# libnxz/power-gzip

Hardware: AMD Instinct MI355X
Metric: GiB/s uncompressed in (deflate), real-data corpus in 64 KiB blocks, exact dynamic-Huffman table per block (higher is better)
Workload: dtype u8

## Files before the change

### power-gzip_amd/csrc/nxz_batch.cpp

```cpp
#include "nxz_ctx.h"
#include "nxz_inflate_part.h"

static size_t compress_chunk(size_t n)
{
	static const size_t v = [] { const char *e = getenv("NXZ_COMPRESS_CHUNK"); size_t x = e ? (size_t)strtoull(e, nullptr, 0) : 0; return x >= 256 ? x : (size_t)0; }();
	if (v) return v;
	size_t c = 8192;
	while (c < 65536 && n >= 8 * c) c *= 2;
	return c;
}

static constexpr unsigned JOB_COUNTERS = 256;
#define NXZ_LANES_MIN 49152
static_assert(NXZ_INFLATE_PART_CHUNK_STREAMS < NXZ_LANES_MIN, "a chunk of nxz_batch_inflate_streams_part must stay below the batches that are sampled or go a stream per lane");
#define NXZ_LANES_TABLES_MIN 163840
#define NXZ_WINDOW_LDS_MAX 1024
#define NXZ_DICT_WG_MIN_DEFAULT 4096

extern "C" int nxz_dict_create(nxz_ctx_t *c, const uint8_t *bytes, size_t len, nxz_dict_t **out)
{
	if (!c || !out || (len && !bytes)) return -EINVAL;
	if (forked_child()) return -ENODEV;
	(void)hipSetDevice(c->device);
	nxz_dict *d = new (std::nothrow) nxz_dict;
	if (!d) return -ENOMEM;
	d->device = c->device; d->len = len;
	d->id = nxz_dict_adler32(bytes, len);
	d->win = nxz_dict_inflate_window(len); d->W = nxz_dict_deflate_window(len);
	std::vector<uint8_t> img(NXZ_DICT_WINDOW, 0);
	if (d->win) memcpy(img.data() + NXZ_DICT_WINDOW - d->win, bytes + nxz_dict_inflate_start(len), d->win);
	if (hipMalloc((void **)&d->d_win, NXZ_DICT_WINDOW) != hipSuccess) { (void)hipGetLastError(); delete d; return -ENOMEM; }
	hipError_t e = hipMemcpy(d->d_win, img.data(), NXZ_DICT_WINDOW, hipMemcpyHostToDevice);
	if (e != hipSuccess) { set_err("dictionary copy", e); (void)hipFree(d->d_win); delete d; return -EIO; }
	*out = d;
	return 0;
}
extern "C" void nxz_dict_destroy(nxz_ctx_t *c, nxz_dict_t *d)
{
	if (!d) return;
	if (!forked_child()) { (void)hipSetDevice(d->device); (void)hipFree(d->d_win); }
	delete d;
}
extern "C" uint32_t nxz_dict_id(const nxz_dict_t *d) { return d ? d->id : 1; }

static int batch_compress(nxz_ctx_t *c, int fc, const nxz_batch_job_t *jobs, size_t n,
			  const nxz_batch_dht_t *dht, size_t ntables, nxz_batch_result_t *results,
			  uint32_t *counts, void *stream, const nxz_dict *dict, const uint8_t *win = nullptr, size_t nwin = 0);
extern "C" int nxz_batch_compress(nxz_ctx_t *c, int fc, const nxz_batch_job_t *jobs, size_t n,
				  const nxz_batch_dht_t *dht, size_t ntables, nxz_batch_result_t *results,
				  uint32_t *counts, void *stream)
{
	return batch_compress(c, fc, jobs, n, dht, ntables, results, counts, stream, nullptr);
}
extern "C" int nxz_batch_compress_dict(nxz_ctx_t *c, int fc, const nxz_dict_t *dict, const nxz_batch_job_t *jobs, size_t n,
				       const nxz_batch_dht_t *dht, size_t ntables, nxz_batch_result_t *results,
				       uint32_t *counts, void *stream)
{
	if (!c || !dict || dict->device != c->device || n >= (1u << 31) || (n && (!jobs || !results))) return -EINVAL;
	return batch_compress(c, fc, jobs, n, dht, ntables, results, counts, stream, dict);
}
int batch_compress_windowed(nxz_ctx_t *c, int fc, const uint8_t *win, size_t nwin, const nxz_batch_job_t *jobs, size_t n,
			    nxz_batch_result_t *results, void *stream)
{
	if (!win || nwin > n) return -EINVAL;
	return batch_compress(c, fc, jobs, n, nullptr, 0, results, nullptr, stream, nullptr, win, nwin);
}
static int batch_compress(nxz_ctx_t *c, int fc, const nxz_batch_job_t *ujobs, size_t n,
			  const nxz_batch_dht_t *dht, size_t ntables, nxz_batch_result_t *results,
			  uint32_t *counts, void *stream, const nxz_dict *dict, const uint8_t *win, size_t nwin)
{
	const nxz_batch_job_t *jobs = ujobs;
	if (!c || !nxz_fc_is_compress((uint32_t)fc) || (fc & 1) || (fc & ~0x2e)) return -EINVAL;
	if (forked_child()) return -ENODEV;
	const bool gen = nxz_fc_is_dhtgen((uint32_t)fc);
	const bool isdht = nxz_fc_is_dht((uint32_t)fc), count = nxz_fc_has_count((uint32_t)fc);
	if (gen && !isdht) return -EINVAL;
	if (count && !counts) return -EINVAL;
	if (isdht && !gen && (!dht || !ntables)) return -EINVAL;
	if (n == 0) return 0;
	hipStream_t s = (hipStream_t)stream;
	(void)hipSetDevice(c->device);
	nxz_dht_prepared_t *prepared = nullptr;
	const char *fge = getenv("NXZ_FUSED_GEN");
	const bool fused_gen_on = fge && atoi(fge) != 0;
	const bool fused_gen = gen && fused_gen_on;
	const bool fused = (!isdht && !count) || fused_gen;
	size_t want = compress_chunk(n);
	size_t nchunks = fused ? 1 : (n + want - 1) / want;
	size_t chunk = (n + nchunks - 1) / nchunks;
	nxz_ctx::Scratch sc;
	const auto use = lease_scratch(c, s);
	const int sized = with_scratch(c, s, [&](nxz_ctx::Scratch &r) -> int {
		if (!fused && r.chunk_limit && want > r.chunk_limit) {
			want = r.chunk_limit; nchunks = (n + want - 1) / want; chunk = (n + nchunks - 1) / nchunks;
		}
		if (!fused && r.chunk_cap < chunk) {
			if (r.d_tokens) { (void)hipStreamSynchronize(s); r.release_chunk(); }
			const size_t per_job = (size_t)NXZ_TOK_STRIDE + sizeof(nxz_dht_prepared_t) + 316 * sizeof(uint32_t);
			size_t free_b = 0, total_b = 0;
			if (hipMemGetInfo(&free_b, &total_b) == hipSuccess && want > 8192 && chunk * per_job > free_b / 4) {
				while (want > 8192 && want * per_job > free_b / 4) want /= 2;
				nchunks = (n + want - 1) / want; chunk = (n + nchunks - 1) / nchunks;
				r.chunk_limit = want;
			}
			while (!r.alloc_chunk(chunk)) {
				if (want <= 1024) return -ENOMEM;
				want = want > 8192 ? 8192 : want / 2;
				nchunks = (n + want - 1) / want; chunk = (n + nchunks - 1) / nchunks;
				r.chunk_limit = want;
			}
		}
		if (!r.d_cand2) HIPCHK(hipMalloc((void **)&r.d_cand2, nxz_lz77_cand2_bytes()), return -ENOMEM);
		if (fused_gen && !r.d_fuse) HIPCHK(hipMalloc((void **)&r.d_fuse, nxz_lz77_gen_scratch_bytes()), return -ENOMEM);
		if (isdht && !gen && r.buf[BUF_PREPARED].grow(s, ntables * sizeof(nxz_dht_prepared_t)) == DevBuf::FAILED) return -ENOMEM;
		if (!c->d_job_counters && hipMalloc((void **)&c->d_job_counters, JOB_COUNTERS * sizeof(uint32_t)) != hipSuccess) c->d_job_counters = nullptr;
		if (dict && r.buf[BUF_DICT_JOBS].grow(s, n * sizeof(nxz_batch_job_t)) == DevBuf::FAILED) return -ENOMEM;
		sc = r;
		return 0;
	});
	if (sized) return sized;
	if (dict) {
		nxz_batch_job_t *djobs = sc.buf[BUF_DICT_JOBS].as<nxz_batch_job_t>();
		if (int rc = launched("dictionary jobs launch", nxz_launch_dict_jobs(ujobs, n, dict->W, djobs, s))) return rc;
		jobs = djobs;
	}
	if (isdht && !gen) {
		prepared = sc.buf[BUF_PREPARED].as<nxz_dht_prepared_t>();
		if (int rc = launched("dht prepare launch", nxz_launch_dht_prepare(dht, ntables, prepared, s))) return rc;
	}
	if (dict) { win = dict->deflate_window(); nwin = n; }
	for (size_t off = 0; off < n; off += chunk) {
		const size_t m = n - off < chunk ? n - off : chunk;
		const size_t mw = off < nwin ? std::min(m, nwin - off) : 0;
		auto draw = [&]() {
			std::lock_guard<std::mutex> g(c->mtx);
			return c->d_job_counters ? c->d_job_counters + (c->next_counter++ % JOB_COUNTERS) : nullptr;
		};
		uint32_t *cnt = count ? counts + off * 316 : gen ? sc.d_counts : nullptr;
		auto stamp = [&]() {
			if (!c->timing) return;
			hipEvent_t e;
			if (hipEventCreate(&e) != hipSuccess) return;
			(void)hipEventRecord(e, s);
			std::lock_guard<std::mutex> g(c->mtx);
			c->tev.push_back(e);
		};
		stamp();
		const int mode = fused_gen ? NXZ_LZ77_FUSED_GEN : fused ? NXZ_LZ77_FUSED_FHT : cnt != nullptr;
		uint8_t *const lz_scratch = fused_gen ? sc.d_fuse : sc.d_tokens;
		uint32_t *const lz_counts = fused_gen && !count ? nullptr : cnt;
		int rc = mw ? nxz_launch_lz77_dict(mode, jobs + off, mw, lz_scratch, sc.d_cand2, results + off, lz_counts, draw(), win, s) : 0;
		if (!rc && mw < m)
			rc = nxz_launch_lz77(mode, jobs + off + mw, m - mw, fused ? lz_scratch : lz_scratch + mw * (size_t)NXZ_TOK_STRIDE, sc.d_cand2,
					     results + off + mw, lz_counts ? lz_counts + mw * 316 : nullptr, draw(), s);
		if ((rc = launched("lz77 launch", rc)) != 0) return rc;
		stamp();
		if (fused) { stamp(); stamp(); continue; }
		if (gen) {
			if ((rc = launched("dhtgen launch", nxz_launch_dhtgen(cnt, m, sc.d_gen, nullptr, s))) != 0) return rc;
		}
		stamp();
		rc = launched("encode launch", nxz_launch_encode(isdht, gen, jobs + off, m, sc.d_tokens, gen ? sc.d_gen : prepared, results + off, s));
		if (rc) return rc;
		stamp();
	}
	return dict ? launched("dictionary finish launch", nxz_launch_dict_finish(ujobs, n, dict->W, results, s)) : 0;
}

size_t trim_compress_scratch()
{
	size_t freed = 0;
	std::lock_guard<std::mutex> g(g_mtx);
	for (nxz_ctx *c : g_ctx) {
		if (!c) continue;
		(void)hipSetDevice(c->device);
		std::vector<std::pair<hipStream_t, std::mutex *>> streams;
		{
			std::lock_guard<std::mutex> g2(c->mtx);
			for (auto &kv : c->scratch) streams.emplace_back(kv.first, &c->scratch_use[kv.first]);
		}
		for (auto &sm : streams) {
			if (!sm.second->try_lock()) continue;
			bool there;
			{
				std::lock_guard<std::mutex> g2(c->mtx);
				there = c->scratch.find(sm.first) != c->scratch.end();
			}
			if (there && hipStreamSynchronize(sm.first) != hipSuccess) { (void)hipGetLastError(); there = false; }
			if (there) {
				std::lock_guard<std::mutex> g2(c->mtx);
				auto it = c->scratch.find(sm.first);
				if (it != c->scratch.end()) {
					nxz_ctx::Scratch &r = it->second;
					if (r.d_tokens) freed += r.chunk_cap * ((size_t)NXZ_TOK_STRIDE + sizeof(nxz_dht_prepared_t) + 316 * sizeof(uint32_t));
					r.release_chunk();
					r.chunk_limit = 0;
				}
			}
			sm.second->unlock();
		}
	}
	return freed;
}

extern "C" void nxz_ctx_stage_timing(nxz_ctx_t *c, int on)
{
	if (!c) return;
	std::lock_guard<std::mutex> g(c->mtx);
	c->timing = on != 0;
}

extern "C" int nxz_ctx_stage_ms(nxz_ctx_t *c, double ms[3], unsigned *launches)
{
	if (!c || !ms) return -EINVAL;
	std::vector<hipEvent_t> ev;
	{
		std::lock_guard<std::mutex> g(c->mtx);
		ev.swap(c->tev);
	}
	ms[0] = ms[1] = ms[2] = 0;
	if (launches) *launches = (unsigned)(ev.size() / 4);
	for (size_t i = 0; i + 3 < ev.size(); i += 4) {
		(void)hipEventSynchronize(ev[i + 3]);
		for (int k = 0; k < 3; k++) {
			float f = 0;
			if (hipEventElapsedTime(&f, ev[i + k], ev[i + k + 1]) == hipSuccess) ms[k] += f;
		}
	}
	for (auto e : ev) (void)hipEventDestroy(e);
	return 0;
}

extern "C" int nxz_batch_dhtgen(nxz_ctx_t *c, const uint32_t *counts, size_t n, nxz_batch_dht_t *tables, void *stream)
{
	if (!c || !counts || !tables) return -EINVAL;
	if (forked_child()) return -ENODEV;
	(void)hipSetDevice(c->device);
	return launched("dhtgen launch", nxz_launch_dhtgen(counts, n, nullptr, tables, (hipStream_t)stream));
}

extern "C" int nxz_batch_decompress(nxz_ctx_t *c, const nxz_batch_job_t *jobs, size_t n,
// ... 238 lines not shown
```

### power-gzip_amd/csrc/nxz_device.h

```cpp
#ifndef NXZ_DEVICE_H
#define NXZ_DEVICE_H
#include <stdint.h>
#include <stddef.h>
#include "../../include/nxz_engine.h"

typedef struct nxz_dht_prepared {
	uint32_t dhtlen;
	uint32_t status;
	uint32_t dhtw[74];
	uint32_t ll[288];
	uint32_t d[32];
} nxz_dht_prepared_t;

#define NXZ_TOK_LITBITS    0u
#define NXZ_TOK_MATCHBITS  8192u
#define NXZ_TOK_RECORDS    16384u
#define NXZ_TOK_STRIDE     106496u
#define NXZ_TOK_MAXREC     ((NXZ_TOK_STRIDE - NXZ_TOK_RECORDS) / 4u)

#ifdef __HIPCC__
#include <hip/hip_runtime.h>
#define NXZ_GLOBAL_AS __attribute__((address_space(1)))
extern "C" {
#define NXZ_LZ77_MAX_GRID 512
#define NXZ_LZ77_FUSED_FHT 2
#define NXZ_LZ77_FUSED_GEN 3
size_t nxz_lz77_cand2_bytes(void);
size_t nxz_lz77_gen_scratch_bytes(void);
int nxz_launch_lz77(int count, const nxz_batch_job_t *jobs, size_t n, uint8_t *tokens, uint16_t *cand2, nxz_batch_result_t *results,
		    uint32_t *counts, uint32_t *job_counter, hipStream_t stream);
int nxz_launch_symcount(const nxz_batch_job_t *jobs, size_t n, const uint8_t *tokens, uint32_t *counts, hipStream_t stream);
int nxz_launch_encode(int dht, int table_per_job, const nxz_batch_job_t *jobs, size_t n, const uint8_t *tokens,
		      const nxz_dht_prepared_t *tables, nxz_batch_result_t *results, hipStream_t stream);
int nxz_launch_dhtgen(const uint32_t *counts, size_t n, nxz_dht_prepared_t *prepared,
		      nxz_batch_dht_t *tables, hipStream_t stream);
int nxz_launch_dht_prepare(const nxz_batch_dht_t *dht, size_t n, nxz_dht_prepared_t *out, hipStream_t stream);
int nxz_launch_wrap(const nxz_batch_job_t *jobs, size_t n, nxz_batch_result_t *results, hipStream_t stream);
int nxz_launch_wrap_sliced(const nxz_batch_job_t *jobs, size_t n, nxz_batch_result_t *results, hipStream_t stream);
int nxz_launch_inflate(const nxz_batch_job_t *jobs, size_t n, nxz_batch_result_t *results,
		       nxz_batch_dht_t *dht_io, int window_in_lds, const uint32_t *order, hipStream_t stream);
size_t nxz_order_workspace(size_t n);
const uint32_t *nxz_launch_order_by_length(const nxz_batch_job_t *jobs, size_t n, uint8_t *workspace, hipStream_t stream);
typedef struct nxz_sync_req {
	const uint8_t *src;
	uint32_t srclen;
	uint32_t header_bit;
	uint32_t guess_bit;
	uint32_t limit_bit;
} nxz_sync_req_t;
typedef struct nxz_sync_res { uint32_t bit; uint32_t lanes; } nxz_sync_res_t;
size_t nxz_built_tables_bytes(void);
#define NXZ_BLOCKFIND_MORE 3u
int nxz_launch_token_sync_more(const nxz_sync_req_t *breqs, uint32_t nb, nxz_batch_dht_t *tables, void *built, uint32_t first,
			       const nxz_sync_req_t *reqs, uint32_t n, nxz_sync_res_t *res, hipStream_t stream);
int nxz_launch_token_sync(const nxz_sync_req_t *breqs, uint32_t nb, nxz_batch_dht_t *tables, void *built,
			  const nxz_sync_req_t *reqs, uint32_t n, nxz_sync_res_t *res, hipStream_t stream);
typedef struct nxz_walk_req { const uint8_t *src; uint64_t src_len; uint64_t bit; uint32_t rem, bfinal; } nxz_walk_req_t;
typedef struct nxz_walk_res { uint64_t bit; uint32_t flags, reserved; } nxz_walk_res_t;
int nxz_launch_stored_walk(const nxz_walk_req_t *reqs, uint32_t n, nxz_walk_res_t *res, hipStream_t stream);
int nxz_launch_inflate_w16(const nxz_batch_job_t *jobs, size_t n, nxz_batch_result_t *results, nxz_batch_dht_t *dht_io, const void *built,
			   int few_and_even, hipStream_t stream);
int nxz_launch_sample_btype(const nxz_batch_job_t *jobs, size_t n, uint32_t *out, hipStream_t stream);
int nxz_launch_cksum(const nxz_batch_job_t *jobs, size_t n, nxz_batch_result_t *results, hipStream_t stream);
int nxz_launch_pack_stream(const nxz_batch_job_t *jobs, const nxz_batch_result_t *results, size_t n, uint32_t final_index,
			   uint64_t *offsets, uint8_t *packed, hipStream_t stream);
typedef struct nxz_pack_member { uint32_t b0, n, fin, off0; uint8_t *packed; } nxz_pack_member_t;
int nxz_launch_pack_member_streams(const nxz_batch_job_t *jobs, const nxz_batch_result_t *results, size_t nblocks, const nxz_pack_member_t *members,
				   size_t nmembers, const uint16_t *member_of, uint64_t *offsets, hipStream_t stream);
int nxz_launch_copy_items(const void *items, uint32_t n, hipStream_t stream);
int nxz_launch_copy16(const void *src, void *dst, size_t bytes, hipStream_t stream);
size_t nxz_inflate_lanes_workspace(size_t n);
unsigned nxz_inflate_cut_pieces(size_t n);
size_t nxz_inflate_cut_workspace(size_t n, unsigned pieces, size_t arena);
int nxz_launch_copy_out(const nxz_batch_job_t *jobs, const nxz_batch_result_t *results, uint8_t *const *targets, size_t n, hipStream_t stream);
int nxz_launch_inflate_cut(const nxz_batch_job_t *jobs, size_t n, nxz_batch_result_t *results, nxz_batch_dht_t *dht_io,
			   unsigned pieces, uint8_t *workspace, size_t arena, hipStream_t stream);
int nxz_launch_pack_members(const nxz_batch_job_t *jobs, const nxz_batch_result_t *results, size_t n,
			    uint64_t *offsets, uint8_t *packed, hipStream_t stream);
int nxz_launch_pack_zlib(const nxz_batch_job_t *jobs, const nxz_batch_result_t *results, size_t n, uint32_t flg,
			 uint64_t *offsets, uint8_t *packed, hipStream_t stream);
int nxz_launch_frame_header(int fmt, const nxz_batch_job_t *jobs, size_t n, nxz_batch_frame_t *frames, nxz_batch_job_t *derived, hipStream_t stream);
int nxz_launch_frame_trailer(const nxz_batch_job_t *jobs, size_t n, nxz_batch_result_t *results, nxz_batch_frame_t *frames, hipStream_t stream);
size_t nxz_bgzf_workspace(uint64_t len, uint64_t cap);
int nxz_launch_bgzf_discover(const uint8_t *packed, uint64_t len, uint8_t *dst, uint64_t *offsets, uint64_t max_members, uint8_t *ws,
			     uint64_t cap, nxz_batch_job_t **jobs, hipStream_t stream);
int nxz_launch_bgzf_coff(const uint8_t *packed, uint64_t len, uint8_t *ws, uint64_t cap, uint64_t max_members, uint64_t *coff, hipStream_t stream);
size_t nxz_bgzf_ranges_workspace(uint64_t n, uint64_t L);
int nxz_launch_bgzf_map(const uint8_t *packed, uint64_t packed_len, const uint64_t *coff, const uint64_t *uoff, uint64_t L, int kind,
			const nxz_bgzf_range_t *ranges, uint64_t n, uint64_t *offsets, uint32_t *status, uint8_t *ws, hipStream_t stream);
int nxz_launch_range_map_clear(uint8_t *ws, uint64_t n, uint64_t L, hipStream_t stream);
int nxz_launch_range_map_ranges(const uint64_t *uoff, uint64_t L, const nxz_bgzf_range_t *ranges, uint64_t n, uint64_t *offsets,
				uint32_t *status, uint8_t *ws, hipStream_t stream);
void nxz_range_map_lists(uint8_t *ws, uint64_t n, uint64_t L, const uint32_t **midx, const uint32_t **list);
int nxz_launch_bgzf_jobs(const uint8_t *packed, const uint64_t *coff, const uint64_t *uoff, uint64_t n, uint64_t L, uint8_t *ws,
			 uint64_t k0, uint64_t cnt, uint8_t *slots, uint64_t stride, nxz_batch_job_t *jobs, hipStream_t stream);
int nxz_launch_bgzf_gather(const uint64_t *uoff, uint64_t n, uint64_t L, uint64_t pieces, uint8_t *ws, const uint64_t *offsets,
			   const uint8_t *slots, uint64_t stride, uint64_t k0, uint64_t cnt, const nxz_batch_frame_t *frames,
			   const nxz_batch_result_t *results, uint8_t *dst, uint32_t *status, hipStream_t stream);
int nxz_launch_bgzf_zero(uint64_t n, const uint64_t *offsets, const uint32_t *status, uint8_t *dst, hipStream_t stream);
int nxz_launch_inflate_lanes(const nxz_batch_job_t *jobs, size_t n, nxz_batch_result_t *results,
			     nxz_batch_dht_t *dht_io, uint8_t *workspace, int init_fixed, hipStream_t stream);
size_t nxz_inflate_wg_workspace(size_t n);
int nxz_launch_inflate_wg(const nxz_batch_job_t *jobs, size_t n, nxz_batch_result_t *results, nxz_batch_dht_t *dht_io,
			  uint8_t *wg_ws, const uint32_t *order, uint8_t *const *targets, hipStream_t stream);
int nxz_launch_cksum_copy(const nxz_batch_job_t *jobs, size_t n, nxz_batch_result_t *results, uint8_t *const *targets, hipStream_t stream);
int nxz_launch_dict_jobs(const nxz_batch_job_t *in, size_t n, uint32_t W, nxz_batch_job_t *out, hipStream_t stream);
int nxz_launch_dict_finish(const nxz_batch_job_t *in, size_t n, uint32_t W, nxz_batch_result_t *results, hipStream_t stream);
int nxz_launch_lz77_dict(int count, const nxz_batch_job_t *jobs, size_t n, uint8_t *tokens, uint16_t *cand2, nxz_batch_result_t *results,
			 uint32_t *counts, uint32_t *job_counter, const uint8_t *dict, hipStream_t stream);
int nxz_launch_inflate_wg_dict(const nxz_batch_job_t *jobs, size_t n, nxz_batch_result_t *results, uint8_t *wg_ws, const uint32_t *order,
			       const uint8_t *dwin, uint32_t dlen, uint32_t src_min, hipStream_t stream);
int nxz_launch_inflate_order_only_dict(const nxz_batch_job_t *jobs, size_t nslots, nxz_batch_result_t *results, const uint32_t *order,
				       const uint8_t *dict_end, uint32_t dlen, uint32_t src_below, hipStream_t stream);
int nxz_launch_pack_zlib_dict(const nxz_batch_job_t *jobs, const nxz_batch_result_t *results, size_t n, uint32_t flg, uint32_t dictid,
// ... 128 lines not shown
```

### power-gzip_amd/csrc/nxz_engine.cpp

```cpp
#include "nxz_ctx.h"

#define NXZ_VERSION "nxz-engine 0.1 (gfx950)"

static thread_local char g_err[256];
void set_err(const char *what, hipError_t e)
{
	snprintf(g_err, sizeof(g_err), "%s: %s", what, e == hipSuccess ? "error" : hipGetErrorString(e));
}

extern "C" const char *nxz_last_error(void) { return g_err; }
extern "C" size_t nxz_pinflate_trim(void);
extern "C" size_t nxz_trim(void) { return nxz_pinflate_trim() + trim_compress_scratch(); }
extern "C" const char *nxz_engine_version(void) { return NXZ_VERSION; }
extern "C" size_t nxz_compress_bound(size_t n) { return ((n * 9 + 7) / 8 + 16 + 15) & ~(size_t)15; }

#define OUT_CAP (SUBBLOCK * 2 + 4096)
#define INF_SRC_CAP (1u << 20)
#define INF_OUT_CAP (4u << 20)

std::mutex g_mtx;
nxz_ctx *g_ctx[64];
pid_t g_creator_pid = 0;

static bool slot_init(Slot &s)
// ... 343 lines not shown
		if (!on || !jobs) return;
		const double j = (double)jobs, r = (double)(rounds ? rounds.load() : 1);
		fprintf(stderr, "nxz job trace: %llu compress jobs in %llu rounds (%.1f per round); per job: slot %.1f us, gather %.1f us, in the round %.1f us, "
			"scatter %.1f us; per round: launch calls %.1f us, synchronise %.1f us\n", (unsigned long long)jobs, (unsigned long long)rounds, j / r,
			ns_acquire / j * 1e-3, ns_gather / j * 1e-3, ns_wait / j * 1e-3, ns_finish / j * 1e-3, ns_issue / r * 1e-3, ns_sync / r * 1e-3);
	}
} g_trace;

struct CompressReq {
	uint32_t fc = 0;
	nxz_batch_job_t job;
	const nxz_cpb_t *cpb = nullptr;
	nxz_batch_result_t res;
	uint32_t cnt[316];
	int rc = 0;
	bool taken = false, done = false;
};
#define ROUND_MAX 32u

static void round_free(nxz_ctx::Round &r)
{
	if (r.stream) (void)hipStreamDestroy(r.stream);
	if (r.h_jobs) (void)hipHostFree(r.h_jobs);
	if (r.h_res) (void)hipHostFree(r.h_res);
	if (r.h_dht) (void)hipHostFree(r.h_dht);
	if (r.h_cnt) (void)hipHostFree(r.h_cnt);
	if (r.h_items) (void)hipHostFree(r.h_items);
	if (r.d_prep) (void)hipFree(r.d_prep);
	if (r.d_tok) (void)hipFree(r.d_tok);
	if (r.d_cand2) (void)hipFree(r.d_cand2);
	if (r.d_src) (void)hipFree(r.d_src);
	if (r.d_cut) (void)hipFree(r.d_cut);
	if (r.d_wg) (void)hipFree(r.d_wg);
	if (r.h_targets) (void)hipHostFree(r.h_targets);
	const bool busy = r.busy;
	r = nxz_ctx::Round();
	r.busy = busy;
}

static bool round_init(nxz_ctx::Round &r)
{
	if (r.ready) return true;
	static std::atomic<unsigned> round_turn{0};
	auto fail = [&]() { round_free(r); return false; };
	HIPCHK(stream_create_spread(&r.stream, round_turn.fetch_add(1)), return fail());
	HIPCHK(hipHostMalloc((void **)&r.h_jobs, ROUND_MAX * sizeof(nxz_batch_job_t)), return fail());
	HIPCHK(hipHostMalloc((void **)&r.h_res, ROUND_MAX * sizeof(nxz_batch_result_t)), return fail());
	HIPCHK(hipHostMalloc((void **)&r.h_dht, ROUND_MAX * sizeof(nxz_batch_dht_t)), return fail());
	HIPCHK(hipHostMalloc((void **)&r.h_cnt, ROUND_MAX * 316 * sizeof(uint32_t)), return fail());
	HIPCHK(hipMalloc((void **)&r.d_prep, ROUND_MAX * sizeof(nxz_dht_prepared_t)), return fail());
	HIPCHK(hipMalloc((void **)&r.d_tok, (size_t)ROUND_MAX * NXZ_TOK_STRIDE), return fail());
	HIPCHK(hipMalloc((void **)&r.d_cand2, nxz_lz77_cand2_bytes() / NXZ_LZ77_MAX_GRID * ROUND_MAX), return fail());
	HIPCHK(hipMalloc((void **)&r.d_src, (size_t)ROUND_MAX * SUBBLOCK), return fail());
	HIPCHK(hipHostMalloc((void **)&r.h_items, ROUND_MAX * sizeof(nxz_ctx::Round::Item)), return fail());
	r.ready = true;
	return true;
}

static int round_run(nxz_ctx *c, nxz_ctx::Round &R, std::vector<CompressReq *> &v)
{
	const uint32_t fc = v[0]->fc;
	const size_t n = v.size();
	const bool dht = nxz_fc_is_dht(fc), count = nxz_fc_has_count(fc), gen = nxz_fc_is_dhtgen(fc);
	(void)hipSetDevice(c->device);
	const uint64_t t0 = g_trace.on ? trace_ns() : 0;
	for (size_t k = 0; k < n; k++) {
		R.h_jobs[k] = v[k]->job;
		R.h_jobs[k].dht_index = (uint32_t)k;
		R.h_items[k].src = v[k]->job.src; R.h_items[k].dst = R.d_src + k * (size_t)SUBBLOCK; R.h_items[k].bytes = v[k]->job.src_len;
		R.h_jobs[k].src = R.h_items[k].dst;
		if (dht && !gen) {
			R.h_dht[k].dhtlen = nxz_in_dhtlen(v[k]->cpb);
			memcpy(R.h_dht[k].dht, v[k]->cpb->in_dht, NXZ_DHT_MAXSZ);
		}
	}
	static const bool each = getenv("NXZ_JOB_TRACE") && atoi(getenv("NXZ_JOB_TRACE")) > 1;
	static std::atomic<uint64_t> kns[4];
	auto lap = [&](int i, uint64_t from) { if (each) { (void)hipStreamSynchronize(R.stream); kns[i] += trace_ns() - from; } };
	uint64_t k0 = each ? trace_ns() : 0;
	if (nxz_launch_copy_items(R.h_items, (uint32_t)n, R.stream)) return -EIO;
	if (dht && !gen && nxz_launch_dht_prepare(R.h_dht, n, R.d_prep, R.stream)) return -EIO;
	lap(0, k0); k0 = each ? trace_ns() : 0;
	const bool fused = !dht && !count && !gen;
	if (nxz_launch_lz77(fused ? NXZ_LZ77_FUSED_FHT : count || gen, R.h_jobs, n, R.d_tok, R.d_cand2, R.h_res, R.h_cnt, nullptr, R.stream)) return -EIO;
	lap(1, k0); k0 = each ? trace_ns() : 0;
	if (gen && nxz_launch_dhtgen(R.h_cnt, n, R.d_prep, nullptr, R.stream)) return -EIO;
	lap(2, k0); k0 = each ? trace_ns() : 0;
	if (!fused && nxz_launch_encode(dht, gen, R.h_jobs, n, R.d_tok, R.d_prep, R.h_res, R.stream)) return -EIO;
	lap(3, k0);
	if (each && (g_trace.rounds & 255) == 255)
		fprintf(stderr, "nxz round kernels (sum so far, us): dht_prepare %.0f lz77 %.0f dhtgen %.0f encode %.0f over %llu rounds\n",
			kns[0] * 1e-3, kns[1] * 1e-3, kns[2] * 1e-3, kns[3] * 1e-3, (unsigned long long)g_trace.rounds + 1);
	const uint64_t t1 = g_trace.on ? trace_ns() : 0;
	HIPCHK(hipStreamSynchronize(R.stream), return -EIO);
	if (g_trace.on) { g_trace.rounds++; g_trace.ns_issue += t1 - t0; g_trace.ns_sync += trace_ns() - t1; }
	for (size_t k = 0; k < n; k++) {
		v[k]->res = R.h_res[k];
		if (count) memcpy(v[k]->cnt, R.h_cnt + k * 316, sizeof(v[k]->cnt));
	}
	return 0;
}

static nxz_ctx::Round *free_round(nxz_ctx *c, bool inflate = false)
{
	static const unsigned limit_c = [] { const char *e = getenv("NXZ_ROUNDS"); unsigned v = e ? (unsigned)atoi(e) : 6; return v < 1 ? 1u : v > 16 ? 16u : v; }();
	static const unsigned limit_i = [] { const char *e = getenv("NXZ_ROUNDS_INFLATE"); unsigned v = e ? (unsigned)atoi(e) : getenv("NXZ_ROUNDS") ? (unsigned)atoi(getenv("NXZ_ROUNDS")) : 3; return v < 1 ? 1u : v > 16 ? 16u : v; }();
	const unsigned limit = inflate ? limit_i : limit_c;
	unsigned busy = 0;
	nxz_ctx::Round *f = nullptr;
	for (auto &r : c->rounds) { if (r.busy) busy++; else if (!f) f = &r; }
	return busy < limit ? f : nullptr;
}

static int round_submit(nxz_ctx *c, CompressReq *me)
{
	std::unique_lock<std::mutex> lk(c->qm);
	c->q.push_back(me);
	while (!me->done) {
		nxz_ctx::Round *R = nullptr;
		if (!me->taken) R = free_round(c);
		if (!R) { c->qcv.wait(lk); continue; }
		R->busy = true;
		std::vector<CompressReq *> v;
		const uint32_t fc = c->q.front()->fc;
		for (auto it = c->q.begin(); it != c->q.end() && v.size() < ROUND_MAX; ) {
			if ((*it)->fc == fc) { (*it)->taken = true; v.push_back(*it); it = c->q.erase(it); }
			else ++it;
		}
		lk.unlock();
		(void)hipSetDevice(c->device);
		int rc = round_init(*R) ? round_run(c, *R, v) : -ENOMEM;
		if (rc && R->stream) (void)hipStreamSynchronize(R->stream);
		lk.lock();
		for (auto *r : v) { r->rc = rc; r->done = true; }
		R->busy = false;
		c->qcv.notify_all();
	}
	return me->rc;
}

static int run_compress(nxz_ctx *c, Slot *s, nxz_crb_cpb_t *j, uint32_t fc)
{
	uint32_t srctotal = nxz_dde_bytes(&j->crb.source);
	uint32_t hist = nxz_fc_is_resume(fc) ? nxz_in_histlen(&j->cpb) * 16 : 0;
	if (hist > srctotal) hist = srctotal;
	uint32_t skip = hist > 32768 ? hist - 32768 : 0;
	uint32_t h = hist - skip;
	uint32_t n = srctotal - hist;
	bool partial = false;
	if (h + n > SUBBLOCK) { n = SUBBLOCK - h; partial = true; }
	const uint64_t t0 = g_trace.on ? trace_ns() : 0;
	uint32_t got = dde_gather(&j->crb.source, skip, s->h_in, h + n);
	if (got < h) { h = got; n = 0; } else n = got - h;
	uint32_t cap = dde_capacity(&j->crb.target);
	uint32_t dcap = cap < OUT_CAP ? cap & ~3u : OUT_CAP;
	if (cap < 4) dcap = 0;
	const bool count = nxz_fc_has_count(fc);

	CompressReq req;
	req.fc = fc;
	req.cpb = &j->cpb;
	memset(&req.job, 0, sizeof(req.job));
	req.job.src = s->h_in; req.job.dst = s->h_out; req.job.src_len = h + n; req.job.hist_len = h;
	req.job.dst_cap = dcap; req.job.in_crc = nxz_in_crc(&j->cpb); req.job.in_adler = nxz_in_adler(&j->cpb);
	const uint64_t t1 = g_trace.on ? trace_ns() : 0;
	int rc = round_submit(c, &req);
	if (rc) return rc;
	const uint64_t t2 = g_trace.on ? trace_ns() : 0;

// ... 253 lines not shown
```

### power-gzip_amd/csrc/nxz_symcount.hip

```cpp
#include <hip/hip_runtime.h>
#include <stdint.h>
#include "nxz_device.h"
#include "nxz_symcount.h"

namespace nxzsc {

constexpr int NT = (int)LANES;
constexpr int NW = NT / 64;
constexpr uint32_t HSTRIDE = 320;
constexpr uint32_t GROUP = 4;

typedef uint32_t v4u __attribute__((ext_vector_type(4)));

__global__ __launch_bounds__(NT) void count_kernel(const nxz_batch_job_t *__restrict__ jobs_, const uint8_t *__restrict__ tokens_,
						    uint32_t *__restrict__ counts_, uint32_t njobs)
{
	__shared__ uint32_t hist[NW][HSTRIDE];
	__shared__ uint32_t wsum[NW];
	const int t = threadIdx.x, lane = t & 63, wave = t >> 6;
	const uint32_t bid = blockIdx.x;
	if (bid >= njobs) return;
	const nxz_batch_job_t job = jobs_[bid];
	const uint32_t total = job.src_len;
	const uint32_t h = job.hist_len < total ? job.hist_len : total;
	const uint32_t n = total - h < BLOCK_MAX ? total - h : BLOCK_MAX;
	const uint8_t NXZ_GLOBAL_AS *src = (const uint8_t NXZ_GLOBAL_AS *)job.src + h;
	const uint8_t NXZ_GLOBAL_AS *tk = (const uint8_t NXZ_GLOBAL_AS *)tokens_ + (size_t)bid * NXZ_TOK_STRIDE;
	const uint32_t NXZ_GLOBAL_AS *litb = (const uint32_t NXZ_GLOBAL_AS *)(tk + NXZ_TOK_LITBITS);
	const uint32_t NXZ_GLOBAL_AS *tokb = (const uint32_t NXZ_GLOBAL_AS *)(tk + NXZ_TOK_MATCHBITS);
	const uint32_t NXZ_GLOBAL_AS *recs = (const uint32_t NXZ_GLOBAL_AS *)(tk + NXZ_TOK_RECORDS);
	uint32_t NXZ_GLOBAL_AS *out = (uint32_t NXZ_GLOBAL_AS *)counts_ + (size_t)bid * NSYM;
	const uint32_t nwords = (n + 31) >> 5;

	struct Fetch { uint64_t bytes[GROUP]; uint32_t litw[GROUP]; };
	auto fetch = [&](uint32_t r0, Fetch &f) {
#pragma unroll
		for (uint32_t j = 0; j < GROUP; j++) {
			const uint32_t p0 = r0 + j * RPOS + 8 * t;
			f.bytes[j] = 0; f.litw[j] = 0;
			if (p0 < n) {
				f.litw[j] = litb[p0 >> 5];
				f.bytes[j] = lane_bytes(src, p0, n);
			}
		}
	};

	uint32_t s = 0;
	{
		const v4u NXZ_GLOBAL_AS *tw = (const v4u NXZ_GLOBAL_AS *)tokb;
		v4u a = { 0, 0, 0, 0 }, b = a;
		if (8u * t < nwords) { a = tw[2 * t]; b = tw[2 * t + 1]; }
		const uint32_t w[8] = { a.x, a.y, a.z, a.w, b.x, b.y, b.z, b.w };
#pragma unroll
		for (int k = 0; k < 8; k++) s += (uint32_t)__popc(w[k] & word_mask(8u * t + k, n));
	}
	Fetch nx;
	fetch(0, nx);
	for (uint32_t i = t; i < NW * HSTRIDE; i += NT) (&hist[0][0])[i] = 0;
	for (int o = 32; o > 0; o >>= 1) s += __shfl_down(s, o, 64);
	if (lane == 0) wsum[wave] = s;
	__syncthreads();
	uint32_t nrec = 0;
#pragma unroll
	for (int w = 0; w < NW; w++) nrec += wsum[w];
	if (nrec > NXZ_TOK_MAXREC) nrec = NXZ_TOK_MAXREC;
	uint32_t *my = hist[wave];

	for (uint32_t i0 = 0; i0 < nrec; i0 += 4 * NT) {
		uint32_t r[4];
#pragma unroll
		for (int j = 0; j < 4; j++) {
			const uint32_t i = i0 + NT * j + t;
			r[j] = i < nrec ? recs[i] : 0;
		}
#pragma unroll
		for (int j = 0; j < 4; j++) {
			if (i0 + NT * j + t < nrec) {
				uint32_t ls, ds;
				record_symbols(r[j], ls, ds);
				atomicAdd(&my[ls], 1u);
				atomicAdd(&my[ds], 1u);
			}
		}
	}

	for (uint32_t r0 = 0; r0 < n; r0 += GROUP * RPOS) {
		const Fetch k = nx;
		if (r0 + GROUP * RPOS < n) fetch(r0 + GROUP * RPOS, nx);
#pragma unroll
		for (uint32_t j = 0; j < GROUP; j++)
			lane_literals(k.bytes[j], k.litw[j], r0 + j * RPOS + 8 * t, n, [&](uint32_t sym) { atomicAdd(&my[sym], 1u); });
	}
	__syncthreads();

	for (uint32_t i = t; i < NSYM; i += NT) {
		uint32_t c = 0;
#pragma unroll
		for (int w = 0; w < NW; w++) c += hist[w][i];
		out[i] = i == EOB ? 1u : c;
	}
}

}

extern "C" int nxz_launch_symcount(const nxz_batch_job_t *jobs, size_t n, const uint8_t *tokens, uint32_t *counts, hipStream_t stream)
{
	if (n == 0) return 0;
	hipLaunchKernelGGL(nxzsc::count_kernel, dim3((unsigned)n), dim3(nxzsc::NT), 0, stream, jobs, tokens, counts, (uint32_t)n);
	return (int)hipGetLastError();
}
```

Before: 109.0.

## Fuse symbol counting with Huffman table generation in one kernel

For the dynamic-Huffman generate path, the LZ77 kernel now emits only tokens (no in-kernel counts). A new kernel counts symbols from the token buffer and builds the DHT in the same workgroup, reusing LDS for the histogram and table-building scratch. This replaces the separate count-in-LZ77 plus dhtgen launch and removes the global round trip of the counts. The cost is an extra read pass over tokens and source bytes, plus table generation running on only one wave per block. An env var restores the old separate path.

```diff
diff --git a/power-gzip_amd/csrc/nxz_batch.cpp b/power-gzip_amd/csrc/nxz_batch.cpp
--- a/power-gzip_amd/csrc/nxz_batch.cpp
+++ b/power-gzip_amd/csrc/nxz_batch.cpp
@@ -85,6 +85,7 @@
 	const bool fused_gen_on = fge && atoi(fge) != 0;
 	const bool fused_gen = gen && fused_gen_on;
 	const bool fused = (!isdht && !count) || fused_gen;
+	const bool count_table = gen && !fused && !nxz_table_separate();
 	size_t want = compress_chunk(n);
 	size_t nchunks = fused ? 1 : (n + want - 1) / want;
 	size_t chunk = (n + nchunks - 1) / nchunks;
@@ -146,9 +147,9 @@
 			c->tev.push_back(e);
 		};
 		stamp();
-		const int mode = fused_gen ? NXZ_LZ77_FUSED_GEN : fused ? NXZ_LZ77_FUSED_FHT : cnt != nullptr;
+		const int mode = fused_gen ? NXZ_LZ77_FUSED_GEN : fused ? NXZ_LZ77_FUSED_FHT : count_table || !cnt ? NXZ_LZ77_TOKENS : NXZ_LZ77_COUNTS;
 		uint8_t *const lz_scratch = fused_gen ? sc.d_fuse : sc.d_tokens;
-		uint32_t *const lz_counts = fused_gen && !count ? nullptr : cnt;
+		uint32_t *const lz_counts = (fused_gen && !count) || count_table ? nullptr : cnt;
 		int rc = mw ? nxz_launch_lz77_dict(mode, jobs + off, mw, lz_scratch, sc.d_cand2, results + off, lz_counts, draw(), win, s) : 0;
 		if (!rc && mw < m)
 			rc = nxz_launch_lz77(mode, jobs + off + mw, m - mw, fused ? lz_scratch : lz_scratch + mw * (size_t)NXZ_TOK_STRIDE, sc.d_cand2,
@@ -156,7 +157,10 @@
 		if ((rc = launched("lz77 launch", rc)) != 0) return rc;
 		stamp();
 		if (fused) { stamp(); stamp(); continue; }
-		if (gen) {
+		if (count_table) {
+			rc = nxz_launch_count_table(jobs + off, m, sc.d_tokens, count ? cnt : nullptr, sc.d_gen, nullptr, s);
+			if ((rc = launched("count and table launch", rc)) != 0) return rc;
+		} else if (gen) {
 			if ((rc = launched("dhtgen launch", nxz_launch_dhtgen(cnt, m, sc.d_gen, nullptr, s))) != 0) return rc;
 		}
 		stamp();
diff --git a/power-gzip_amd/csrc/nxz_counttable.hip b/power-gzip_amd/csrc/nxz_counttable.hip
--- /dev/null
+++ b/power-gzip_amd/csrc/nxz_counttable.hip
@@ -0,0 +1,62 @@
+#include <hip/hip_runtime.h>
+#include <stdint.h>
+#include <stdlib.h>
+#include "nxz_device.h"
+#include "nxz_symcount_dev.h"
+#include "nxz_dhtgen_dev.h"
+
+namespace nxzct {
+
+using nxzsc::NT; using nxzsc::NW; using nxzsc::HSTRIDE; using nxzsc::NSYM; using nxzsc::EOB;
+
+struct NoBar { static constexpr bool none = true; __device__ __forceinline__ void operator()() const {} };
+
+constexpr uint32_t HIST_BYTES = NW * HSTRIDE * 4;
+constexpr uint32_t WORK_BYTES = HIST_BYTES > nxzd::WAVE_LDS ? HIST_BYTES : nxzd::WAVE_LDS;
+static_assert(NSYM == nxzd::NTOT && NSYM <= HSTRIDE, "one layout of the counts");
+
+__global__ __launch_bounds__(NT) __attribute__((amdgpu_waves_per_eu(8, 8))) void count_table_kernel(const nxz_batch_job_t *__restrict__ jobs_, const uint8_t *__restrict__ tokens_,
+							  uint32_t *__restrict__ counts_, nxz_dht_prepared_t *__restrict__ prepared_,
+							  nxz_batch_dht_t *__restrict__ tables_, uint32_t njobs)
+{
+	__shared__ __attribute__((aligned(16))) uint8_t work[WORK_BYTES];
+	__shared__ uint32_t sum[HSTRIDE];
+	__shared__ uint32_t wsum[NW];
+	const int t = threadIdx.x;
+	const uint32_t bid = blockIdx.x;
+	if (bid >= njobs) return;
+	uint32_t (*hist)[HSTRIDE] = (uint32_t (*)[HSTRIDE])work;
+	nxzsc::count_block(hist, wsum, jobs_, tokens_, bid, t);
+
+	for (uint32_t i = t; i < HSTRIDE; i += NT) {
+		uint32_t c = 0;
+#pragma unroll
+		for (int w = 0; w < NW; w++) c += hist[w][i];
+		sum[i] = i == EOB ? 1u : c;
+	}
+	__syncthreads();
+	if (counts_) {
+		uint32_t NXZ_GLOBAL_AS *out = (uint32_t NXZ_GLOBAL_AS *)counts_ + (size_t)bid * NSYM;
+		for (uint32_t i = t; i < NSYM; i += NT) out[i] = sum[i];
+	}
+	if (t >= 64) return;
+
+	NoBar nb;
+	nxzd::dhtgen_wave(work, (const uint32_t *)sum, prepared_ ? prepared_ + bid : nullptr, tables_ ? tables_ + bid : nullptr, t, nb);
+}
+
+}
+
+extern "C" int nxz_table_separate(void)
+{
+	const char *a = getenv("NXZ_TABLE_SEPARATE"), *b = getenv("NXZ_LZ77_COUNT_INKERNEL");
+	return (a && atoi(a) != 0) || (b && atoi(b) != 0);
+}
+
+extern "C" int nxz_launch_count_table(const nxz_batch_job_t *jobs, size_t n, const uint8_t *tokens, uint32_t *counts,
+				      nxz_dht_prepared_t *prepared, nxz_batch_dht_t *tables, hipStream_t stream)
+{
+	if (n == 0) return 0;
+	hipLaunchKernelGGL(nxzct::count_table_kernel, dim3((unsigned)n), dim3(nxzct::NT), 0, stream, jobs, tokens, counts, prepared, tables, (uint32_t)n);
+	return (int)hipGetLastError();
+}
diff --git a/power-gzip_amd/csrc/nxz_device.h b/power-gzip_amd/csrc/nxz_device.h
--- a/power-gzip_amd/csrc/nxz_device.h
+++ b/power-gzip_amd/csrc/nxz_device.h
@@ -23,6 +23,8 @@
 #define NXZ_GLOBAL_AS __attribute__((address_space(1)))
 extern "C" {
 #define NXZ_LZ77_MAX_GRID 512
+#define NXZ_LZ77_TOKENS 0
+#define NXZ_LZ77_COUNTS 1
 #define NXZ_LZ77_FUSED_FHT 2
 #define NXZ_LZ77_FUSED_GEN 3
 size_t nxz_lz77_cand2_bytes(void);
@@ -30,6 +32,9 @@
 int nxz_launch_lz77(int count, const nxz_batch_job_t *jobs, size_t n, uint8_t *tokens, uint16_t *cand2, nxz_batch_result_t *results,
 		    uint32_t *counts, uint32_t *job_counter, hipStream_t stream);
 int nxz_launch_symcount(const nxz_batch_job_t *jobs, size_t n, const uint8_t *tokens, uint32_t *counts, hipStream_t stream);
+int nxz_launch_count_table(const nxz_batch_job_t *jobs, size_t n, const uint8_t *tokens, uint32_t *counts,
+			   nxz_dht_prepared_t *prepared, nxz_batch_dht_t *tables, hipStream_t stream);
+int nxz_table_separate(void);
 int nxz_launch_encode(int dht, int table_per_job, const nxz_batch_job_t *jobs, size_t n, const uint8_t *tokens,
 		      const nxz_dht_prepared_t *tables, nxz_batch_result_t *results, hipStream_t stream);
 int nxz_launch_dhtgen(const uint32_t *counts, size_t n, nxz_dht_prepared_t *prepared,
diff --git a/power-gzip_amd/csrc/nxz_engine.cpp b/power-gzip_amd/csrc/nxz_engine.cpp
--- a/power-gzip_amd/csrc/nxz_engine.cpp
+++ b/power-gzip_amd/csrc/nxz_engine.cpp
@@ -449,9 +449,12 @@
 	if (dht && !gen && nxz_launch_dht_prepare(R.h_dht, n, R.d_prep, R.stream)) return -EIO;
 	lap(0, k0); k0 = each ? trace_ns() : 0;
 	const bool fused = !dht && !count && !gen;
-	if (nxz_launch_lz77(fused ? NXZ_LZ77_FUSED_FHT : count || gen, R.h_jobs, n, R.d_tok, R.d_cand2, R.h_res, R.h_cnt, nullptr, R.stream)) return -EIO;
+	const bool count_table = gen && !nxz_table_separate();
+	const int mode = fused ? NXZ_LZ77_FUSED_FHT : (count || gen) && !count_table ? NXZ_LZ77_COUNTS : NXZ_LZ77_TOKENS;
+	if (nxz_launch_lz77(mode, R.h_jobs, n, R.d_tok, R.d_cand2, R.h_res, R.h_cnt, nullptr, R.stream)) return -EIO;
 	lap(1, k0); k0 = each ? trace_ns() : 0;
-	if (gen && nxz_launch_dhtgen(R.h_cnt, n, R.d_prep, nullptr, R.stream)) return -EIO;
+	if (count_table ? nxz_launch_count_table(R.h_jobs, n, R.d_tok, count ? R.h_cnt : nullptr, R.d_prep, nullptr, R.stream)
+			: gen && nxz_launch_dhtgen(R.h_cnt, n, R.d_prep, nullptr, R.stream)) return -EIO;
 	lap(2, k0); k0 = each ? trace_ns() : 0;
 	if (!fused && nxz_launch_encode(dht, gen, R.h_jobs, n, R.d_tok, R.d_prep, R.h_res, R.stream)) return -EIO;
 	lap(3, k0);
diff --git a/power-gzip_amd/csrc/nxz_symcount.hip b/power-gzip_amd/csrc/nxz_symcount.hip
--- a/power-gzip_amd/csrc/nxz_symcount.hip
+++ b/power-gzip_amd/csrc/nxz_symcount.hip
@@ -1,97 +1,20 @@
 #include <hip/hip_runtime.h>
 #include <stdint.h>
 #include "nxz_device.h"
-#include "nxz_symcount.h"
+#include "nxz_symcount_dev.h"
 
 namespace nxzsc {
-
-constexpr int NT = (int)LANES;
-constexpr int NW = NT / 64;
-constexpr uint32_t HSTRIDE = 320;
-constexpr uint32_t GROUP = 4;
-
-typedef uint32_t v4u __attribute__((ext_vector_type(4)));
 
 __global__ __launch_bounds__(NT) void count_kernel(const nxz_batch_job_t *__restrict__ jobs_, const uint8_t *__restrict__ tokens_,
 						    uint32_t *__restrict__ counts_, uint32_t njobs)
 {
 	__shared__ uint32_t hist[NW][HSTRIDE];
 	__shared__ uint32_t wsum[NW];
-	const int t = threadIdx.x, lane = t & 63, wave = t >> 6;
+	const int t = threadIdx.x;
 	const uint32_t bid = blockIdx.x;
 	if (bid >= njobs) return;
-	const nxz_batch_job_t job = jobs_[bid];
-	const uint32_t total = job.src_len;
-	const uint32_t h = job.hist_len < total ? job.hist_len : total;
-	const uint32_t n = total - h < BLOCK_MAX ? total - h : BLOCK_MAX;
-	const uint8_t NXZ_GLOBAL_AS *src = (const uint8_t NXZ_GLOBAL_AS *)job.src + h;
-	const uint8_t NXZ_GLOBAL_AS *tk = (const uint8_t NXZ_GLOBAL_AS *)tokens_ + (size_t)bid * NXZ_TOK_STRIDE;
-	const uint32_t NXZ_GLOBAL_AS *litb = (const uint32_t NXZ_GLOBAL_AS *)(tk + NXZ_TOK_LITBITS);
-	const uint32_t NXZ_GLOBAL_AS *tokb = (const uint32_t NXZ_GLOBAL_AS *)(tk + NXZ_TOK_MATCHBITS);
-	const uint32_t NXZ_GLOBAL_AS *recs = (const uint32_t NXZ_GLOBAL_AS *)(tk + NXZ_TOK_RECORDS);
 	uint32_t NXZ_GLOBAL_AS *out = (uint32_t NXZ_GLOBAL_AS *)counts_ + (size_t)bid * NSYM;
-	const uint32_t nwords = (n + 31) >> 5;
-
-	struct Fetch { uint64_t bytes[GROUP]; uint32_t litw[GROUP]; };
-	auto fetch = [&](uint32_t r0, Fetch &f) {
-#pragma unroll
-		for (uint32_t j = 0; j < GROUP; j++) {
-			const uint32_t p0 = r0 + j * RPOS + 8 * t;
-			f.bytes[j] = 0; f.litw[j] = 0;
-			if (p0 < n) {
-				f.litw[j] = litb[p0 >> 5];
-				f.bytes[j] = lane_bytes(src, p0, n);
-			}
-		}
-	};
-
-	uint32_t s = 0;
-	{
-		const v4u NXZ_GLOBAL_AS *tw = (const v4u NXZ_GLOBAL_AS *)tokb;
-		v4u a = { 0, 0, 0, 0 }, b = a;
-		if (8u * t < nwords) { a = tw[2 * t]; b = tw[2 * t + 1]; }
-		const uint32_t w[8] = { a.x, a.y, a.z, a.w, b.x, b.y, b.z, b.w };
-#pragma unroll
-		for (int k = 0; k < 8; k++) s += (uint32_t)__popc(w[k] & word_mask(8u * t + k, n));
-	}
-	Fetch nx;
-	fetch(0, nx);
-	for (uint32_t i = t; i < NW * HSTRIDE; i += NT) (&hist[0][0])[i] = 0;
-	for (int o = 32; o > 0; o >>= 1) s += __shfl_down(s, o, 64);
-	if (lane == 0) wsum[wave] = s;
-	__syncthreads();
-	uint32_t nrec = 0;
-#pragma unroll
-	for (int w = 0; w < NW; w++) nrec += wsum[w];
-	if (nrec > NXZ_TOK_MAXREC) nrec = NXZ_TOK_MAXREC;
-	uint32_t *my = hist[wave];
-
-	for (uint32_t i0 = 0; i0 < nrec; i0 += 4 * NT) {
-		uint32_t r[4];
-#pragma unroll
-		for (int j = 0; j < 4; j++) {
-			const uint32_t i = i0 + NT * j + t;
-			r[j] = i < nrec ? recs[i] : 0;
-		}
-#pragma unroll
-		for (int j = 0; j < 4; j++) {
-			if (i0 + NT * j + t < nrec) {
-				uint32_t ls, ds;
-				record_symbols(r[j], ls, ds);
-				atomicAdd(&my[ls], 1u);
-				atomicAdd(&my[ds], 1u);
-			}
-		}
-	}
-
-	for (uint32_t r0 = 0; r0 < n; r0 += GROUP * RPOS) {
-		const Fetch k = nx;
-		if (r0 + GROUP * RPOS < n) fetch(r0 + GROUP * RPOS, nx);
-#pragma unroll
-		for (uint32_t j = 0; j < GROUP; j++)
-			lane_literals(k.bytes[j], k.litw[j], r0 + j * RPOS + 8 * t, n, [&](uint32_t sym) { atomicAdd(&my[sym], 1u); });
-	}
-	__syncthreads();
+	count_block(hist, wsum, jobs_, tokens_, bid, t);
 
 	for (uint32_t i = t; i < NSYM; i += NT) {
 		uint32_t c = 0;
diff --git a/power-gzip_amd/csrc/nxz_symcount_dev.h b/power-gzip_amd/csrc/nxz_symcount_dev.h
--- /dev/null
+++ b/power-gzip_amd/csrc/nxz_symcount_dev.h
@@ -0,0 +1,95 @@
+#ifndef NXZ_SYMCOUNT_DEV_H
+#define NXZ_SYMCOUNT_DEV_H
+#include <hip/hip_runtime.h>
+#include <stdint.h>
+#include "nxz_device.h"
+#include "nxz_symcount.h"
+
+namespace nxzsc {
+
+constexpr int NT = (int)LANES;
+constexpr int NW = NT / 64;
+constexpr uint32_t HSTRIDE = 320;
+constexpr uint32_t GROUP = 4;
+
+typedef uint32_t v4u __attribute__((ext_vector_type(4)));
+
+__device__ __forceinline__ void count_block(uint32_t (*hist)[HSTRIDE], uint32_t *wsum, const nxz_batch_job_t *__restrict__ jobs_,
+					    const uint8_t *__restrict__ tokens_, const uint32_t bid, const int t)
+{
+	const int lane = t & 63, wave = t >> 6;
+	const nxz_batch_job_t job = jobs_[bid];
+	const uint32_t total = job.src_len;
+	const uint32_t h = job.hist_len < total ? job.hist_len : total;
+	const uint32_t n = total - h < BLOCK_MAX ? total - h : BLOCK_MAX;
+	const uint8_t NXZ_GLOBAL_AS *src = (const uint8_t NXZ_GLOBAL_AS *)job.src + h;
+	const uint8_t NXZ_GLOBAL_AS *tk = (const uint8_t NXZ_GLOBAL_AS *)tokens_ + (size_t)bid * NXZ_TOK_STRIDE;
+	const uint32_t NXZ_GLOBAL_AS *litb = (const uint32_t NXZ_GLOBAL_AS *)(tk + NXZ_TOK_LITBITS);
+	const uint32_t NXZ_GLOBAL_AS *tokb = (const uint32_t NXZ_GLOBAL_AS *)(tk + NXZ_TOK_MATCHBITS);
+	const uint32_t NXZ_GLOBAL_AS *recs = (const uint32_t NXZ_GLOBAL_AS *)(tk + NXZ_TOK_RECORDS);
+	const uint32_t nwords = (n + 31) >> 5;
+
+	struct Fetch { uint64_t bytes[GROUP]; uint32_t litw[GROUP]; };
+	auto fetch = [&](uint32_t r0, Fetch &f) {
+#pragma unroll
+		for (uint32_t j = 0; j < GROUP; j++) {
+			const uint32_t p0 = r0 + j * RPOS + 8 * t;
+			f.bytes[j] = 0; f.litw[j] = 0;
+			if (p0 < n) {
+				f.litw[j] = litb[p0 >> 5];
+				f.bytes[j] = lane_bytes(src, p0, n);
+			}
+		}
+	};
+
+	uint32_t s = 0;
+	{
+		const v4u NXZ_GLOBAL_AS *tw = (const v4u NXZ_GLOBAL_AS *)tokb;
+		v4u a = { 0, 0, 0, 0 }, b = a;
+		if (8u * t < nwords) { a = tw[2 * t]; b = tw[2 * t + 1]; }
+		const uint32_t w[8] = { a.x, a.y, a.z, a.w, b.x, b.y, b.z, b.w };
+#pragma unroll
+		for (int k = 0; k < 8; k++) s += (uint32_t)__popc(w[k] & word_mask(8u * t + k, n));
+	}
+	Fetch nx;
+	fetch(0, nx);
+	for (uint32_t i = t; i < NW * HSTRIDE; i += NT) (&hist[0][0])[i] = 0;
+	for (int o = 32; o > 0; o >>= 1) s += __shfl_down(s, o, 64);
+	if (lane == 0) wsum[wave] = s;
+	__syncthreads();
+	uint32_t nrec = 0;
+#pragma unroll
+	for (int w = 0; w < NW; w++) nrec += wsum[w];
+	if (nrec > NXZ_TOK_MAXREC) nrec = NXZ_TOK_MAXREC;
+	uint32_t *my = hist[wave];
+
+	for (uint32_t i0 = 0; i0 < nrec; i0 += 4 * NT) {
+		uint32_t r[4];
+#pragma unroll
+		for (int j = 0; j < 4; j++) {
+			const uint32_t i = i0 + NT * j + t;
+			r[j] = i < nrec ? recs[i] : 0;
+		}
+#pragma unroll
+		for (int j = 0; j < 4; j++) {
+			if (i0 + NT * j + t < nrec) {
+				uint32_t ls, ds;
+				record_symbols(r[j], ls, ds);
+				atomicAdd(&my[ls], 1u);
+				atomicAdd(&my[ds], 1u);
+			}
+		}
+	}
+
+	for (uint32_t r0 = 0; r0 < n; r0 += GROUP * RPOS) {
+		const Fetch k = nx;
+		if (r0 + GROUP * RPOS < n) fetch(r0 + GROUP * RPOS, nx);
+#pragma unroll
+		for (uint32_t j = 0; j < GROUP; j++)
+			lane_literals(k.bytes[j], k.litw[j], r0 + j * RPOS + 8 * t, n, [&](uint32_t sym) { atomicAdd(&my[sym], 1u); });
+	}
+	__syncthreads();
+}
+
+}
+#endif
```

Result: no change. 108.9, median of 2 (-0.1%).
